# scientificcomputing/networks_fenicsx

Hardware: NVIDIA B200
Metric: tree-network assemble+solve DOFs/s (higher is better)
Workload: dtype f64

## Files before the change

networks_fenicsx_b200/csrc/assemble.cuh:

```cuda
#pragma once

#include "ctx.cuh"

namespace nxfx {

struct FastDiv {
  uint32_t magic, shift;
};
inline FastDiv make_fastdiv(uint32_t d) {
  FastDiv f;
  uint32_t fl = 31;
  while (!((d >> fl) & 1u)) --fl;
  if ((d & (d - 1)) == 0) {
    f.magic = 0;
    f.shift = fl == 0 ? 0 : fl - 1;
  } else {
    const uint64_t n = 1ull << (32 + fl);
    uint64_t m = n / d;
    const uint64_t rem = n % d;
    m += m;
    if (2 * rem >= d) m += 1;
    f.magic = (uint32_t)(m + 1);
    f.shift = fl;
  }
// ... 266 lines not shown
    for (int k = d.i0; k < d.i1; ++k) {
      const bool in = g.bif_inc[k] & 1;
      put(true, p, in ? 0.0 : -1.0);
      put(true, p + 1, in ? 1.0 : 0.0);
      p += 2;
    }
    if (rhs && !ACC) b[r] = 0.0;
  }
}

constexpr int kFluxRowsN1 = 512;
constexpr int kAsmCap = 2560;
constexpr int kPresRows = 512;
constexpr int kLamRows = 256;

#define NXFX_ST2(ptr, v) __stcs((ptr), (v))
#define NXFX_ST1(ptr, v) __stcs((ptr), (v))
#define NXFX_LDS(ptr) __ldcs(ptr)
#define NXFX_STB2(ptr, v) __stcs((ptr), (v))
#define NXFX_STB1(ptr, v) __stcs((ptr), (v))

template <bool ACC>
__device__ __forceinline__ void store_pair(double* __restrict__ vals, size_t idx, double v0, double v1) {
  if ((idx & 1) == 0) {
    double2* dst = reinterpret_cast<double2*>(vals + idx);
    double2 v = make_double2(v0, v1);
    if (ACC) { const double2 o = *dst; v.x += o.x; v.y += o.y; }
    NXFX_ST2(dst, v);
  } else {
    if (ACC) { vals[idx] += v0; vals[idx + 1] += v1; } else { vals[idx] = v0; vals[idx + 1] = v1; }
  }
}

template <bool ACC>
__device__ __forceinline__ void flush_tile(const double* sm, double* __restrict__ vals, int sbase, int tnnz) {
  const int off = sbase & 1;
  double* out = vals + sbase - off;
  const int lo = off, hi = off + tnnz;
  const int npair = (hi + 1) >> 1;
  for (int q = threadIdx.x; q < npair; q += blockDim.x) {
    const int i = 2 * q;
    if (i >= lo && i + 1 < hi) {
      double2 v = *reinterpret_cast<const double2*>(sm + i);
      double2* dst = reinterpret_cast<double2*>(out + i);
      if (ACC) { const double2 o = *dst; v.x += o.x; v.y += o.y; }
      NXFX_ST2(dst, v);
    } else {
      if (i >= lo && i < hi) { if (ACC) out[i] += sm[i]; else out[i] = sm[i]; }
      if (i + 1 >= lo && i + 1 < hi) { if (ACC) out[i + 1] += sm[i + 1]; else out[i + 1] = sm[i + 1]; }
    }
  }
}

template <bool ACC>
__device__ __forceinline__ void flux_tile_n1(const Net& g, const Coef& c, const int32_t* __restrict__ rowptr,
                                             double* __restrict__ vals, double* __restrict__ b, int lhs,
                                             int rhs, int tile, double* sm) {
  __shared__ int warp_nl[kTileRows / 32];
  const int r0 = tile * kFluxRowsN1;
  const int slot = (r0 >> 1) + threadIdx.x;
  const bool active = slot < g.E;
  const int lane = threadIdx.x & 31, w = threadIdx.x >> 5;
  int4 t = make_int4(0, 0, -1, -1);
  VertexRec v0, v1;
  if (active) {
    const int2 uv = NXFX_LDS(g.slot_uv + slot);
    v0 = load_vertex(g.x2, uv.x);
    v1 = load_vertex(g.x2, uv.y);
    t = make_int4(uv.x, uv.y, lm_unbox(v0.p), lm_unbox(v1.p));
  }
  const bool hu = t.z >= 0, hv = t.w >= 0;
  const unsigned bu = __ballot_sync(0xffffffffu, hu), bv = __ballot_sync(0xffffffffu, hv);
  const unsigned lt = (1u << lane) - 1u;
  int pre = __popc(bu & lt) + __popc(bv & lt);
  if (lane == 0) warp_nl[w] = __popc(bu) + __popc(bv);
  const int sbase = rowptr[r0];
  double m = 0.0;
  if (active) {
    const double R = c.R_cell ? c.R_cell[NXFX_LDS(g.slot_edge + slot)] : c.R_const;
    m = __dmul_rn(R, seg_length(v0, v1));
  }
  __syncthreads();
  int tot = 0;
#pragma unroll
  for (int k = 0; k < kTileRows / 32; ++k) {
    const int v = warp_nl[k];
    if (k < w) pre += v;
    tot += v;
  }
  const int nact = min(kFluxRowsN1 >> 1, g.E - (r0 >> 1));
  const int tnnz = 6 * nact + 2 * tot;
  if (active) {
    const int r = 2 * slot;
    if (rhs) {
      const double b0 = hu ? 0.0 : -v0.p, b1 = hv ? 0.0 : v1.p;
      double2* dst = reinterpret_cast<double2*>(b + r);
      double2 v = make_double2(b0, b1);
      if (ACC) { const double2 o = *dst; v.x += o.x; v.y += o.y; }
      NXFX_STB2(dst, v);
    }
    if (lhs) {
      if (ACC) c.cell_rh[slot] += m; else NXFX_STB1(c.cell_rh + slot, m);
      const double m3 = __dmul_rn(m, kThird), m6 = __dmul_rn(m, kSixth);
      const bool ufirst = !hv || (hu && t.z < t.w);
      const int nl = (int)hu + (int)hv;
      const double u0 = (hu && ufirst) ? -1.0 : 0.0, u1 = ufirst ? 0.0 : -1.0;
      const double w0 = (hu && ufirst) ? 0.0 : 1.0, w1 = ufirst ? 1.0 : 0.0;
      double* s0 = sm + (sbase & 1) + 6 * (int)threadIdx.x + 2 * pre;
      double* s1 = s0 + 3 + nl;
      s0[0] = m3; s0[1] = m6; s0[2] = 1.0;
      s1[0] = m6; s1[1] = m3; s1[2] = -1.0;
      if (nl > 0) { s0[3] = u0; s1[3] = w0; }
      if (nl > 1) { s0[4] = u1; s1[4] = w1; }
    }
  }
  if (lhs) {
    __syncthreads();
    flush_tile<ACC>(sm, vals, sbase, tnnz);
  }
}

template <bool ACC>
__device__ __forceinline__ void flux_tile_gen(const Net& g, const Coef& c, const int32_t* __restrict__ rowptr,
                                              double* __restrict__ vals, double* __restrict__ b, int lhs,
                                              int rhs, int tile, double* sm) {
  const int r0 = tile * kTileRows;
  const int rend = min(r0 + kTileRows, g.nq);
  const int r = r0 + threadIdx.x;
  RowDesc d;
  d.sbase = rowptr[r0];
  d.tnnz = rowptr[rend] - d.sbase;
  d.start = 0; d.a = 0; d.e = 0; d.i0 = d.i1 = 0;
  d.t = make_int4(0, 0, -1, -1);
  const bool active = r < rend;
  if (active) {
    d.start = rowptr[r] - d.sbase;
    const int slot = fastdiv(r, g.div_np1);
    d.a = r - slot * (g.N + 1);
    d.t = g.slot_uvl[slot];
    d.e = g.slot_edge[slot];
  }
  const int lane = threadIdx.x & 31;
  const int rr = active ? r : g.ndofs;
  if (d.tnnz > kAsmCap) {
    if (lhs) assemble_row<ACC, false>(g, c, d, rr, d.sbase + d.start, lane, b, lhs, rhs, GlobalSink<ACC>{vals});
    else assemble_row<ACC, false>(g, c, d, rr, 0, lane, b, lhs, rhs, [](bool, int, double) {});
    return;
  }
  assemble_row<ACC, false>(g, c, d, rr, (d.sbase & 1) + d.start, lane, b, lhs, rhs, SmemSink{sm});
  if (lhs) {
    __syncthreads();
    flush_tile<ACC>(sm, vals, d.sbase, d.tnnz);
  }
}

template <bool ACC, bool N1>
__device__ __forceinline__ void pressure_tile(const Net& g, const Coef& c, const int32_t* __restrict__ rowptr,
                                              double* __restrict__ vals, double* __restrict__ b, int lhs,
                                              int rhs, int tile) {
  const int r0 = g.poff + tile * kPresRows;
  const int rend = min(r0 + kPresRows, g.loff);
// ... 68 lines not shown
```

networks_fenicsx_b200/csrc/nxfx_b200.cu:

```cuda

#include <cub/device/device_scan.cuh>

#include <algorithm>
#include <atomic>
#include <chrono>
#include <cmath>
#include <cstdlib>

#include "assemble.cuh"
#include "ctx.cuh"
#include "condense.cuh"
#include "generic.cuh"
#include "precond.cuh"
#include "spmv.cuh"

using namespace nxfx;

namespace {

constexpr int kScalPartials = 8 * kMaxPartials;
constexpr int kScalSlots = 1024;

Net make_net(const nxfx_ctx* c) {
  Net g;
// ... 453 lines not shown
int cond_backward_local(nxfx_ctx* ctx, double* z, bool add) {
  Net g = make_net(ctx);
  CondDev c = make_cond(ctx);
  TreeDev t = make_tree(ctx);
  const int nb = ctx->tree.n_chunks - 1;
  if (ctx->n_bif > 0 && nb > 0) NXFX_LAUNCH(ctx, btree_sweep_kernel<2>, nb, 1024, 0, t, c, 0);
  const int grid = (int)cdiv((int64_t)ctx->E + ctx->n_bif, kCondThreads);
  if (add) NXFX_LAUNCH(ctx, cond_backsub_kernel<true>, grid, kCondThreads, 0, g, t, c, z);
  else NXFX_LAUNCH(ctx, cond_backsub_kernel<false>, grid, kCondThreads, 0, g, t, c, z);
  return NXFX_OK;
}

int do_cond_apply(nxfx_ctx* ctx, const double* r, double* z, bool add) {
  NXFX_REQUIRE(ctx, ctx->pc_ready, "pc_setup has not been run");
  int rc = cond_forward_local(ctx, r, nullptr);
  if (rc) return rc;
  if (ctx->n_bif > 0) NXFX_LAUNCH(ctx, btree_sweep_kernel<3>, 1, 1024, 0, make_tree(ctx), make_cond(ctx), ctx->tree.n_chunks - 1);
  return cond_backward_local(ctx, z, add);
}

bool n1_kernels(const nxfx_ctx* ctx) { return ctx->N == 1 && ctx->tree.fast_ok; }

int check_aligned(nxfx_ctx* ctx, const double* r, const double* z = nullptr) {
  NXFX_REQUIRE(ctx, (reinterpret_cast<uintptr_t>(r) & 15) == 0 && (reinterpret_cast<uintptr_t>(z) & 15) == 0,
               "vectors must be 16-byte aligned");
  return NXFX_OK;
}

int node_diag(nxfx_ctx* ctx, bool bif) {
  if (n1_kernels(ctx)) {
    if (bif) NXFX_LAUNCH(ctx, bif_diag_n1_kernel, (int)cdiv(ctx->n_bif, kThreads), kThreads, 0, make_net(ctx), make_tree(ctx), ctx->cur->cell_rh.p);
    return NXFX_OK;
  }
  NXFX_LAUNCH(ctx, edge_conductance_kernel, (int)cdiv(ctx->E, kThreads), kThreads, 0, ctx->E, ctx->N, ctx->cur->cell_rh.p, ctx->edge_g.p);
  if (bif) NXFX_LAUNCH(ctx, bif_diag_kernel, (int)cdiv(ctx->n_bif, kThreads), kThreads, 0, make_net(ctx), make_tree(ctx), ctx->edge_g.p);
  return NXFX_OK;
}

int node_rhs(nxfx_ctx* ctx, const double* r, bool bif) {
  Net g = make_net(ctx);
  TreeDev t = make_tree(ctx);
  if (n1_kernels(ctx)) {
    if (bif) NXFX_LAUNCH(ctx, bif_rhs_n1_kernel, (int)cdiv(ctx->n_bif, kThreads), kThreads, 0, g, t, r, ctx->cur->cell_rh.p, ctx->lam_weight.p);
    return NXFX_OK;
  }
  NXFX_LAUNCH(ctx, edge_condense_kernel<false>, (int)cdiv(ctx->E, kThreads), kThreads, 0, g, ctx->cur->cell_rh.p, r,
              ctx->edge_c.p, ctx->edge_fn.p, nullptr);
  if (bif)
    NXFX_LAUNCH(ctx, bif_rhs_kernel<false>, (int)cdiv(ctx->n_bif, kThreads), kThreads, 0, g, t, r, ctx->edge_g.p, ctx->edge_c.p,
                ctx->edge_fn.p, ctx->lam_weight.p);
  return NXFX_OK;
}

int edge_backsub(nxfx_ctx* ctx, const double* r, double* z, bool add, bool pdl = false) {
  Net g = make_net(ctx);
  TreeDev t = make_tree(ctx);
  const double* cell_rh = ctx->cur->cell_rh.p;
  const int grid = (int)cdiv((int64_t)ctx->E + ctx->n_bif, kThreads);
  if (!n1_kernels(ctx)) {
    if (add) NXFX_LAUNCH(ctx, edge_backsub_kernel<true>, grid, kThreads, 0, g, t, cell_rh, r, ctx->edge_g.p, ctx->edge_c.p, z);
    else NXFX_LAUNCH(ctx, edge_backsub_kernel<false>, grid, kThreads, 0, g, t, cell_rh, r, ctx->edge_g.p, ctx->edge_c.p, z);
    return NXFX_OK;
  }
  if (!pdl) {
    if (add) NXFX_LAUNCH(ctx, edge_backsub_n1_kernel<true>, grid, kThreads, 0, g, t, cell_rh, r, z);
    else NXFX_LAUNCH(ctx, edge_backsub_n1_kernel<false>, grid, kThreads, 0, g, t, cell_rh, r, z);
    return NXFX_OK;
  }
  cudaLaunchConfig_t cfg = {};
  cfg.gridDim = dim3((unsigned)grid);
  cfg.blockDim = dim3(kThreads);
  cfg.stream = ctx->stream;
  cudaLaunchAttribute attr[1];
  attr[0].id = cudaLaunchAttributeProgrammaticStreamSerialization;
  attr[0].val.programmaticStreamSerializationAllowed = 1;
  cfg.attrs = attr;
  cfg.numAttrs = 1;
  if (add) NXFX_CUDA(ctx, cudaLaunchKernelEx(&cfg, edge_backsub_n1_kernel<true>, g, t, cell_rh, r, z));
  else NXFX_CUDA(ctx, cudaLaunchKernelEx(&cfg, edge_backsub_n1_kernel<false>, g, t, cell_rh, r, z));
  ctx->launches++;
  return NXFX_OK;
}

int do_pc_setup(nxfx_ctx* ctx) {
  NXFX_REQUIRE(ctx, is_assembled(ctx), "assemble the matrix before pc_setup");
  if (ctx->generic) return do_cond_setup(ctx);
  NXFX_REQUIRE(ctx, ctx->tree.set, "nxfx_set_tree_schedule has not been called");
  const bool n1 = n1_kernels(ctx);
  int rc;
  if (!n1 && (rc = node_diag(ctx, ctx->n_bif > 0))) return rc;
  if (ctx->n_bif > 0 && (rc = tree_pass(ctx, true, nullptr, n1))) return rc;
  mark_factored(ctx);
  return NXFX_OK;
}

bool can_fuse_setup(const nxfx_ctx* ctx) {
  return !ctx->generic && ctx->tree.set && ctx->tree.fast_ok && ctx->tree.coop_fs_ok && ctx->n_bif > 0 &&
         ctx->tree.n_chunks > 1 && (!ctx->lam_weight.p || ctx->comm.ready) && ctx->cur->acc_count == 1;
}

int do_pc_setup_apply(nxfx_ctx* ctx, const double* r, double* z, bool add = false) {
  NXFX_REQUIRE(ctx, is_assembled(ctx), "assemble the matrix before pc_setup");
  const bool n1 = n1_kernels(ctx);
  if (n1) {
    int rc = check_aligned(ctx, r, z);
    if (rc) return rc;
  }
  auto& s = ctx->tree;
  Net g = make_net(ctx);
  TreeDev t = make_tree(ctx);
  FusedN1 fin{g, r, ctx->cur->cell_rh.p, ctx->lam_weight.p};
  unsigned int* tk = ctx->ticket.p + 1;
  unsigned int* fl = ctx->ticket.p + 2;
  unsigned int ep = ++s.epoch;
  int nb = s.n_chunks - 1;
  PeerDev pc = make_peer(ctx, 0);
  if (!n1) {
    NXFX_LAUNCH(ctx, edge_condense_kernel<true>, (int)cdiv(ctx->E, kThreads), kThreads, 0, g, ctx->cur->cell_rh.p, r,
                ctx->edge_c.p, ctx->edge_fn.p, ctx->edge_g.p);
    NXFX_LAUNCH(ctx, bif_rhs_kernel<true>, (int)cdiv(ctx->n_bif, kThreads), kThreads, 0, g, t, r, ctx->edge_g.p,
                ctx->edge_c.p, ctx->edge_fn.p, ctx->lam_weight.p);
    fin.r = nullptr;
    fin.cell_rh = nullptr;
  }
  cudaLaunchConfig_t cfg = {};
  const int gb = std::min(nb, s.coop_fs_blocks - 1);
  cfg.gridDim = dim3(gb + 1);
  cfg.blockDim = dim3(kTreeThreads);
  cfg.dynamicSmemBytes = tree_smem_bytes_fs(s.cap);
  cfg.stream = ctx->stream;
  cudaLaunchAttribute attr[2];
  attr[0].id = cudaLaunchAttributeCooperative;
  attr[0].val.cooperative = 1;
  attr[1].id = cudaLaunchAttributeProgrammaticStreamSerialization;
  attr[1].val.programmaticStreamSerializationAllowed = 1;
  cfg.attrs = attr;
  cfg.numAttrs = ctx->pdl_coop_refused ? 1 : 2;
  const bool multi = gb < nb;
  auto kern = pc.nranks > 1 ? (multi ? tree_factor_solve_coop_kernel<true, true> : tree_factor_solve_coop_kernel<true, false>)
                            : (multi ? tree_factor_solve_coop_kernel<false, true> : tree_factor_solve_coop_kernel<false, false>);
  cudaError_t le = cudaLaunchKernelEx(&cfg, kern, t, nb, tk, fl, ep, fin, pc);
  if (le != cudaSuccess && cfg.numAttrs == 2) {
    cudaGetLastError();
    ctx->pdl_coop_refused = true;
    cfg.numAttrs = 1;
    le = cudaLaunchKernelEx(&cfg, kern, t, nb, tk, fl, ep, fin, pc);
  }
  NXFX_CUDA(ctx, le);
  ctx->launches++;
  mark_factored(ctx);
  return edge_backsub(ctx, r, z, add, true);
}

int do_pc_apply(nxfx_ctx* ctx, int pc_type, const double* r, double* z, bool add = false) {
  const int n = (int)ctx->ndofs;
  if (pc_type == NXFX_PC_NETWORK_SCHUR && ctx->cur->acc_count > 1 && !ctx->pc_unscaled) {
    const size_t ld = vec_stride(ctx);
    if (ctx->work2.n < 2 * ld) {
      NXFX_CUDA(ctx, cudaStreamSynchronize(ctx->stream));
      NXFX_CUDA(ctx, ctx->work2.alloc(2 * ld));
    }
    const double inv_k = 1.0 / (double)ctx->cur->acc_count;
    double* rs = ctx->work2.p;
    double* zs = ctx->work2.p + ld;
    NXFX_LAUNCH(ctx, scale_tail_kernel<false>, vec_grid(ctx, n), kThreads, 0, n, (int)ctx->poff, inv_k, r, rs);
    ctx->pc_unscaled = true;
    const int rc = do_pc_apply(ctx, pc_type, rs, zs, false);
    ctx->pc_unscaled = false;
    if (rc) return rc;
    if (add) NXFX_LAUNCH(ctx, scale_tail_kernel<true>, vec_grid(ctx, n), kThreads, 0, n, (int)ctx->poff, inv_k, zs, z);
    else NXFX_LAUNCH(ctx, scale_tail_kernel<false>, vec_grid(ctx, n), kThreads, 0, n, (int)ctx->poff, inv_k, zs, z);
    return NXFX_OK;
  }
  if (add && pc_type != NXFX_PC_NETWORK_SCHUR) {
    int rc = ensure_work(ctx, 3);
    if (rc) return rc;
    double* tmp = ctx->work.p + 2 * vec_stride(ctx);
    if ((rc = do_pc_apply(ctx, pc_type, r, tmp, false))) return rc;
    NXFX_LAUNCH(ctx, add_kernel, vec_grid(ctx, n), kThreads, 0, n, tmp, z);
    return NXFX_OK;
  }
  if (ctx->comm.ready) {
    NXFX_REQUIRE(ctx, pc_type == NXFX_PC_NETWORK_SCHUR && can_fuse_setup(ctx),
                 "the fused partitioned solve needs a forest schedule that fits the cooperative kernel and pc_type lu");
    return do_pc_setup_apply(ctx, r, z, add);
  }
  if (pc_type == NXFX_PC_NONE) {
    NXFX_CUDA(ctx, cudaMemcpyAsync(z, r, n * sizeof(double), cudaMemcpyDeviceToDevice, ctx->stream));
    return NXFX_OK;
  }
  if (pc_type == NXFX_PC_JACOBI_FLUX) {
    NXFX_LAUNCH(ctx, jacobi_flux_kernel, (int)cdiv(n, kThreads), kThreads, 0, n, (int)ctx->nq,
                ctx->rowptr.p, ctx->colidx.p, ctx->cur->vals.p, r, z);
    return NXFX_OK;
  }
  NXFX_REQUIRE(ctx, ctx->pc_ready, "pc_setup has not been run");
  if (ctx->generic) return do_cond_apply(ctx, r, z, add);
  const bool n1 = n1_kernels(ctx);
  int rc;
  if (n1 && (rc = check_aligned(ctx, r, z))) return rc;
  const bool fuse = n1 && ctx->n_bif > 0 && ctx->tree.coop_ok && ctx->tree.n_chunks > 1 && !ctx->lam_weight.p;
  if ((rc = node_rhs(ctx, r, ctx->n_bif > 0 && !fuse))) return rc;
  if (ctx->n_bif > 0 && (rc = tree_pass(ctx, false, r, fuse))) return rc;
  return edge_backsub(ctx, r, z, add);
}

int factor_bottom(nxfx_ctx* ctx) {
  if (ctx->generic) return cond_factor_local(ctx);
  int rc = node_diag(ctx, true);
  if (rc) return rc;
  const int nb = ctx->tree.n_chunks - 1;
  if (nb > 0) NXFX_LAUNCH(ctx, tree_factor_kernel, nb, kTreeThreads, tree_smem_bytes(ctx->tree.cap), make_tree(ctx), nb, ctx->ticket.p + 1, 0,
                          (FusedN1{make_net(ctx), nullptr, nullptr}));
  return NXFX_OK;
}

int forward_bottom(nxfx_ctx* ctx, const double* r) {
  if (ctx->generic) return cond_forward_local(ctx, r, ctx->lam_weight.p);
  int rc = node_rhs(ctx, r, true);
  if (rc) return rc;
  const int nb = ctx->tree.n_chunks - 1;
  if (nb > 0) NXFX_LAUNCH(ctx, tree_solve_kernel<kTreeUp>, nb, kTreeThreads, tree_smem_bytes(ctx->tree.cap), make_tree(ctx), nb, ctx->ticket.p + 1, 0);
  return NXFX_OK;
}

template <bool FACTOR, int PHASE>
int top_split(nxfx_ctx* ctx, double* buf) {
  const int top = ctx->tree.n_chunks - 1;
  if (!ctx->generic) {
    NXFX_LAUNCH(ctx, (tree_top_kernel<FACTOR, PHASE>), 1, kTreeThreads, tree_smem_bytes(ctx->tree.cap), make_tree(ctx), top, buf);
    return NXFX_OK;
  }
  if (ctx->n_bif == 0) return NXFX_OK;
  const int32_t* idx = ctx->n_shared > 0 ? ctx->top_sh_idx.p : nullptr;
  NXFX_LAUNCH(ctx, (btree_top_split_kernel<FACTOR, PHASE>), 1, 1024, 0, make_tree(ctx), make_cond(ctx), top, idx,
              std::max(ctx->n_shared, 1), buf);
  return NXFX_OK;
}

int backward_bottom(nxfx_ctx* ctx, const double* r, double* z, bool add) {
  if (ctx->generic) return cond_backward_local(ctx, z, add);
  const int nb = ctx->tree.n_chunks - 1;
  if (nb > 0) NXFX_LAUNCH(ctx, tree_solve_kernel<kTreeDown>, nb, kTreeThreads, tree_smem_bytes(ctx->tree.cap), make_tree(ctx), nb, ctx->ticket.p + 1, 0);
  return edge_backsub(ctx, r, z, add);
}

bool fused_split(const nxfx_ctx* ctx) { return !ctx->generic && n1_kernels(ctx); }

int pack_shared(nxfx_ctx* ctx, const double* r, const double* b, double* buf, bool cont) {
  const int ns = ctx->n_shared;
  if (ns == 0) return NXFX_OK;
  NXFX_LAUNCH(ctx, pack_shared_kernel, (int)cdiv(ns, kThreads), kThreads, 0, ns, (int)ctx->loff, ctx->shared_lm.p, r, buf);
  if (!cont) return NXFX_OK;
  NXFX_LAUNCH(ctx, pack_nodal_kernel, (int)cdiv(ns, kThreads), kThreads, 0, ns, (int)ctx->nq, ctx->shared_lm.p, ctx->cond.bif_node.p,
              r, buf + ns);
  NXFX_LAUNCH(ctx, pack_nodal_kernel, (int)cdiv(ns, kThreads), kThreads, 0, ns, (int)ctx->nq, ctx->shared_lm.p, ctx->cond.bif_node.p,
              b, buf + 2 * (size_t)ns);
  return NXFX_OK;
}

inline size_t vec_stride(const nxfx_ctx* ctx) { return ((size_t)ctx->ndofs + 1) & ~(size_t)1; }

int ensure_work(nxfx_ctx* ctx, size_t nvec) {
  const size_t need = nvec * vec_stride(ctx);
  if (ctx->work.n >= need) return NXFX_OK;
  NXFX_CUDA(ctx, cudaStreamSynchronize(ctx->stream));
  NXFX_CUDA(ctx, ctx->work.alloc(need));
  return NXFX_OK;
}

inline double kNormSentinel() {
  const uint64_t bits = 0x7FF8DEADBEEF0001ull;
  double d;
  std::memcpy(&d, &bits, sizeof d);
  return d;
}
inline bool is_norm_sentinel(double v) {
  uint64_t bits;
  std::memcpy(&bits, &v, sizeof bits);
  return bits == 0x7FF8DEADBEEF0001ull;
}
bool poll_norms_enabled() {
  static const bool on = [] { const char* e = std::getenv("NXFX_POLL_NORMS"); return !(e && e[0] == '0'); }();
  return on;
}

void push_history(nxfx_solve_info* info, double v) {
  if (info->history_len < NXFX_HISTORY_LEN) info->history[info->history_len++] = v;
}

int mirror_copy(nxfx_ctx* ctx, const double* x) {
  if (!ctx->mirror_h) return NXFX_OK;
  NXFX_CUDA(ctx, cudaEventRecord(ctx->ev_x, ctx->stream));
  NXFX_CUDA(ctx, cudaStreamWaitEvent(ctx->side, ctx->ev_x, 0));
  NXFX_CUDA(ctx, cudaMemcpyAsync(ctx->mirror_h, x, (size_t)ctx->ndofs * sizeof(double), cudaMemcpyDeviceToHost, ctx->side));
  return NXFX_OK;
}

int solve_preonly(nxfx_ctx* ctx, const double* b, double* x, const nxfx_solve_opts* o, nxfx_solve_info* info,
                  bool fused_setup) {
  int rc = ensure_work(ctx, 3);
  if (rc) return rc;
  double* r = ctx->work.p;
  const int steps = std::max(0, std::min(o->refine_steps, 32));
  if ((rc = fused_setup ? do_pc_setup_apply(ctx, b, x) : do_pc_apply(ctx, o->pc_type, b, x, false))) return rc;
  if ((rc = mirror_copy(ctx, x))) return rc;
  info->iterations = 1;
  if (steps == 0 && !o->final_residual) {
    NXFX_CUDA(ctx, cudaStreamSynchronize(ctx->stream));
    info->rhs_norm = info->residual_norm = -1.0;
    info->converged = 1;
    return NXFX_OK;
  }
  const double rt = o->refine_rtol > 0.0 ? o->refine_rtol : 0.0;
  int applied = 0;
  while (true) {
    const bool lazy = ctx->pipe_ok;
    volatile double* nh = ctx->scal_h;
    const bool poll = poll_norms_enabled();
    if (poll) { ctx->scal_h[0] = kNormSentinel(); ctx->scal_h[1] = kNormSentinel(); }
    if ((rc = do_residual(ctx, b, x, lazy ? nullptr : r, ctx->scal_h_dev, true))) return rc;
    bool arrived = false;
    if (poll) {
      const auto t0 = std::chrono::steady_clock::now();
      for (unsigned spin = 0;; ++spin) {
        if (!is_norm_sentinel(nh[0]) && !is_norm_sentinel(nh[1])) { arrived = true; break; }
        if ((spin & 255u) == 255u && std::chrono::steady_clock::now() - t0 > std::chrono::microseconds(1500)) break;
      }
      std::atomic_thread_fence(std::memory_order_acquire);
    }
    if (!arrived) NXFX_CUDA(ctx, cudaStreamSynchronize(ctx->stream));
    info->rhs_norm = std::sqrt(ctx->scal_h[1]);
    info->residual_norm = std::sqrt(ctx->scal_h[0]);
    push_history(info, info->residual_norm);
    const bool good = std::isfinite(info->residual_norm) && info->residual_norm <= rt * info->rhs_norm;
    if (applied >= steps || (good && rt > 0.0) || !std::isfinite(info->residual_norm)) break;
    if (lazy && (rc = do_residual(ctx, b, x, r, slot(ctx, 0)))) return rc;
    if ((rc = do_pc_apply(ctx, o->pc_type, r, x, true))) return rc;
    if ((rc = mirror_copy(ctx, x))) return rc;
    ++applied;
    if (applied >= steps && !o->final_residual) break;
  }
  info->iterations = 1 + applied;
  const double tol = std::max(o->rtol * info->rhs_norm, o->atol);
  info->converged = std::isfinite(info->residual_norm) && info->residual_norm <= tol;
  return NXFX_OK;
}

int solve_fgmres(nxfx_ctx* ctx, const double* b, double* x, const nxfx_solve_opts* o, nxfx_solve_info* info) {
  const int n = (int)ctx->ndofs;
  const int m = std::max(1, std::min(o->restart > 0 ? o->restart : 30, 200));
  NXFX_REQUIRE(ctx, 2 * (m + 2) + 8 < kScalSlots, "restart too large");
  int rc = ensure_work(ctx, (size_t)(2 * m + 3));
  if (rc) return rc;
  const size_t ld = vec_stride(ctx);
  double* V = ctx->work.p;
  double* Z = V + (size_t)(m + 1) * ld;
  double* w = Z + (size_t)m * ld;
  double* r = w + ld;
  double* hcol = slot(ctx, 8);
  double* hcol2 = slot(ctx, 8 + m + 2);
  double* ycoef = slot(ctx, 8 + 2 * (m + 2));
  std::vector<double> H((size_t)(m + 1) * m, 0.0), cs(m), sn(m), gvec(m + 1), y(m);

  NXFX_CUDA(ctx, cudaMemsetAsync(x, 0, n * sizeof(double), ctx->stream));
  int its = 0;
  const int max_it = o->max_it > 0 ? o->max_it : 10000;
  double tol = 0.0;
  while (true) {
    if ((rc = do_residual(ctx, b, x, r, slot(ctx, 1)))) return rc;
    NXFX_CUDA(ctx, cudaMemcpyAsync(ctx->scal_h, slot(ctx, 1), 2 * sizeof(double), cudaMemcpyDeviceToHost, ctx->stream));
    NXFX_CUDA(ctx, cudaStreamSynchronize(ctx->stream));
    info->rhs_norm = std::sqrt(ctx->scal_h[1]);
    const double beta = std::sqrt(ctx->scal_h[0]);
// ... 1082 lines not shown
```

networks_fenicsx_b200/csrc/precond.cuh:

```cuda
#pragma once

#include "assemble.cuh"
#include "peer.cuh"
#include "spmv.cuh"

namespace nxfx {

struct TreeDev {
  const int32_t* __restrict__ t_of_bif;
  const int32_t* __restrict__ bif_of_t;
  const int32_t* __restrict__ t_parent;
  const int32_t* __restrict__ t_pedge;
  const int32_t* __restrict__ t_pslot;
  const int32_t* __restrict__ t_cptr;
  const int32_t* __restrict__ t_cidx;
  const int32_t* __restrict__ chunk_lptr;
  const int32_t* __restrict__ lvl_ptr;
  const int32_t* __restrict__ chunk_desc;
  const int32_t* __restrict__ t_inc_ptr;
  const int2* __restrict__ t_inc;
  double* diag0;
  double* tg;
  double* d;
  double* gd;
// ... 1048 lines not shown
  const double* rq = r + (size_t)slot * (N + 1);
  const double* rp = r + g.poff + (size_t)e * N;
  const double* rh = cell_rh + (size_t)e * N;
  double* zq = z + (size_t)slot * (N + 1);
  double* zp = z + g.poff + (size_t)e * N;
  const double q0 = edge_g[e] * (edge_c[e] + lu - lv);
  double F = 0.0, qprev = 0.0, qa = q0, hl = 0.0, p = lu;
  for (int a = 0; a <= N; ++a) {
    if (ADD) zq[a] += qa; else zq[a] = qa;
    double qn = 0.0, hr = 0.0;
    if (a < N) {
      F += rp[a];
      qn = q0 + F;
      hr = rh[a];
      const double Mq = hl * (qprev * kSixth + qa * kThird) + hr * (qa * kThird + qn * kSixth);
      p += rq[a] - Mq;
      if (ADD) zp[a] += p; else zp[a] = p;
    }
    qprev = qa;
    qa = qn;
    hl = hr;
  }
}

__global__ void __launch_bounds__(kThreads)
bif_diag_n1_kernel(Net g, TreeDev t, const double* __restrict__ cell_rh) {
  const int i = blockIdx.x * blockDim.x + threadIdx.x;
  if (i >= g.n_bif) return;
  double s = 0.0;
  for (int k = g.bif_ptr[i]; k < g.bif_ptr[i + 1]; ++k) s += 1.0 / cell_rh[g.edge_slot[g.bif_inc[k] >> 1]];
  const int n = t.t_of_bif[i];
  t.diag0[n] = s;
  const int pe = t.t_pslot[n];
  t.tg[n] = pe >= 0 ? 1.0 / cell_rh[pe] : 0.0;
}

__global__ void __launch_bounds__(kThreads)
bif_rhs_n1_kernel(Net g, TreeDev t, const double* __restrict__ r, const double* __restrict__ cell_rh,
                  const double* __restrict__ lam_weight) {
  const int i = blockIdx.x * blockDim.x + threadIdx.x;
  if (i >= g.n_bif) return;
  double s = lam_weight ? -lam_weight[i] * r[g.loff + i] : -r[g.loff + i];
  for (int k = g.bif_ptr[i]; k < g.bif_ptr[i + 1]; ++k) {
    const int inc = g.bif_inc[k], e = inc >> 1;
    const int slot = g.edge_slot[e];
    const double2 rq = *reinterpret_cast<const double2*>(r + 2 * (size_t)slot);
    const double rp = r[g.poff + e], rh = cell_rh[slot];
    const double gc = (1.0 / rh) * (rq.x + rq.y) - 0.5 * rp;
    s += (inc & 1) ? (rp + gc) : -gc;
  }
  t.r[t.t_of_bif[i]] = s;
}

template <bool ADD>
__global__ void __launch_bounds__(kThreads)
edge_backsub_n1_kernel(Net g, TreeDev t, const double* __restrict__ cell_rh, const double* __restrict__ r,
                       double* __restrict__ z) {
  asm volatile("griddepcontrol.launch_dependents;");
  const int idx = blockIdx.x * blockDim.x + threadIdx.x;
  if (idx >= g.E) {
    asm volatile("griddepcontrol.wait;" ::: "memory");
    const int i = idx - g.E;
    if (i < g.n_bif) { if (ADD) z[g.loff + i] += t.lam_nat[i]; else z[g.loff + i] = t.lam_nat[i]; }
    return;
  }
  const int slot = idx;
  const int4 uv = g.slot_uvl[slot];
  const int e = g.slot_edge[slot];
  const double2 rq = *reinterpret_cast<const double2*>(r + 2 * (size_t)slot);
  const double rp = r[g.poff + e], rh = cell_rh[slot];
  asm volatile("griddepcontrol.wait;" ::: "memory");
  const double lu = uv.z >= 0 ? t.lam_nat[uv.z] : 0.0;
  const double lv = uv.w >= 0 ? t.lam_nat[uv.w] : 0.0;
  const double c = (rq.x + rq.y) - 0.5 * rh * rp;
  const double q0 = (c + lu - lv) / rh;
  const double q1 = q0 + rp;
  const double p = lu + rq.x - rh * (q0 * kThird + q1 * kSixth);
  double2* zq = reinterpret_cast<double2*>(z + 2 * (size_t)slot);
  if (ADD) {
    const double2 o = *zq;
    *zq = make_double2(o.x + q0, o.y + q1);
    z[g.poff + e] += p;
  } else {
    *zq = make_double2(q0, q1);
    z[g.poff + e] = p;
  }
}

__global__ void __launch_bounds__(kThreads)
pack_shared_kernel(int n_shared, int loff, const int32_t* __restrict__ shared_lm,
                   const double* __restrict__ v, double* __restrict__ buf) {
  const int i = blockIdx.x * blockDim.x + threadIdx.x;
  if (i < n_shared) buf[i] = v[loff + shared_lm[i]];
}

__global__ void __launch_bounds__(kThreads)
residual_finish_kernel(int n_shared, int loff, const int32_t* __restrict__ shared_lm,
                       const double* __restrict__ buf, double* __restrict__ r, double* __restrict__ nrm_out) {
  __shared__ double red[kThreads / 32];
  double acc = 0.0;
  for (int i = threadIdx.x; i < n_shared; i += blockDim.x) {
    const double v = buf[i];
    r[loff + shared_lm[i]] = v;
    acc += v * v;
  }
  acc = warp_sum(acc);
  if ((threadIdx.x & 31) == 0) red[threadIdx.x >> 5] = acc;
  __syncthreads();
  if (threadIdx.x == 0) {
    double s = buf[n_shared];
    for (int w = 0; w < kThreads / 32; ++w) s += red[w];
    nrm_out[0] = s;
    nrm_out[1] = buf[n_shared + 1];
  }
}

__global__ void __launch_bounds__(kThreads)
jacobi_flux_kernel(int n, int nq, const int32_t* __restrict__ rowptr,
                   const int32_t* __restrict__ colidx, const double* __restrict__ vals,
                   const double* __restrict__ r, double* __restrict__ z) {
  const int i = blockIdx.x * blockDim.x + threadIdx.x;
  if (i >= n) return;
  double v = r[i];
  if (i < nq) {
    for (int k = rowptr[i]; k < rowptr[i + 1]; ++k)
      if (colidx[k] == i) v /= vals[k];
  }
  z[i] = v;
}

}
```

networks_fenicsx_b200/csrc/spmv.cuh:

```cuda
#pragma once

#include "ctx.cuh"
#include "peer.cuh"

namespace nxfx {

constexpr int kEntriesPerThread = kTileCap / kTileRows;
constexpr int kMaxPartials = 4096;

__device__ __forceinline__ double warp_sum(double v) {
#pragma unroll
  for (int o = 16; o > 0; o >>= 1) v += __shfl_down_sync(0xffffffffu, v, o);
  return v;
}

template <int THREADS>
__device__ __forceinline__ double block_sum(double v, double* red ) {
  v = warp_sum(v);
  const int lane = threadIdx.x & 31, w = threadIdx.x >> 5;
  if (lane == 0) red[w] = v;
  __syncthreads();
  double s = 0.0;
  if (w == 0) {
    s = lane < THREADS / 32 ? red[lane] : 0.0;
    s = warp_sum(s);
  }
  __syncthreads();
  return s;
}

template <int THREADS, int K>
__device__ __forceinline__ bool finish_partials(double (&mine)[K], double* partial, int nblocks,
                                                unsigned int* ticket, double* out, double* red) {
  __shared__ bool last;
  if (threadIdx.x == 0) {
#pragma unroll
    for (int k = 0; k < K; ++k) partial[(size_t)k * kMaxPartials + blockIdx.x] = mine[k];
    __threadfence();
    const unsigned int t = atomicAdd(ticket, 1u);
    last = (t == (unsigned int)nblocks - 1);
  }
  __syncthreads();
  if (!last) return false;
  __threadfence();
#pragma unroll
  for (int k = 0; k < K; ++k) {
    double s = 0.0;
    for (int i = threadIdx.x; i < nblocks; i += THREADS)
      s += ((volatile double*)partial)[(size_t)k * kMaxPartials + i];
    s = block_sum<THREADS>(s, red);
    if (threadIdx.x == 0) out[k] = s;
  }
  if (threadIdx.x == 0) *ticket = 0u;
  return true;
}

template <int MODE>
__global__ void __launch_bounds__(kTileRows)
spmv_kernel(int n, int ntiles, const int32_t* __restrict__ rowptr,
            const int32_t* __restrict__ colidx, const double* __restrict__ vals,
            const double* __restrict__ x, double* __restrict__ y, const double* __restrict__ b,
            double* partial, unsigned int* ticket, double* norm2_out) {
  __shared__ double sm[kTileCap];
  __shared__ int srow[kTileRows + 1];
  __shared__ double red[kTileRows / 32];
  double nrm = 0.0, nrb = 0.0;
  for (int tile = blockIdx.x; tile < ntiles; tile += gridDim.x) {
    const int r0 = tile * kTileRows;
    const int nr = min(kTileRows, n - r0);
    if (threadIdx.x <= nr) srow[threadIdx.x] = rowptr[r0 + threadIdx.x];
    if (threadIdx.x == 0) srow[nr] = rowptr[r0 + nr];
    __syncthreads();
    const int sbase = srow[0];
    const int tnnz = srow[nr] - sbase;
    const bool valid = threadIdx.x < nr;
    const int rs = valid ? srow[threadIdx.x] - sbase : 0;
    const int re = valid ? srow[threadIdx.x + 1] - sbase : 0;
    double acc = 0.0;
    for (int c0 = 0; c0 < tnnz; c0 += kTileCap) {
      const int cnt = min(kTileCap, tnnz - c0);
      const size_t g0 = (size_t)sbase + c0;
      double v[kEntriesPerThread];
      int c[kEntriesPerThread];
#pragma unroll
      for (int k = 0; k < kEntriesPerThread; ++k) {
        const int idx = threadIdx.x + k * kTileRows;
        if (idx < cnt) {
          v[k] = __ldg(vals + g0 + idx);
          c[k] = __ldg(colidx + g0 + idx);
        }
      }
#pragma unroll
      for (int k = 0; k < kEntriesPerThread; ++k) {
        const int idx = threadIdx.x + k * kTileRows;
        if (idx < cnt) sm[idx] = __dmul_rn(v[k], x[c[k]]);
      }
      __syncthreads();
      const int s = max(rs - c0, 0), e = min(re - c0, cnt);
      for (int k = s; k < e; ++k) acc = __dadd_rn(acc, sm[k]);
      __syncthreads();
    }
    if (valid) {
      if (MODE == 0) {
        y[r0 + threadIdx.x] = acc;
      } else {
        const double bi = b[r0 + threadIdx.x];
        const double r = __dsub_rn(bi, acc);
        y[r0 + threadIdx.x] = r;
        nrm += r * r;
        nrb += bi * bi;
      }
    }
  }
  if (MODE == 1) {
    double mine[2] = {block_sum<kTileRows>(nrm, red), block_sum<kTileRows>(nrb, red)};
    finish_partials<kTileRows, 2>(mine, partial, gridDim.x, ticket, norm2_out, red);
  }
}

constexpr int kPipeCap = 1792;
#ifndef NXFX_SPMV_STAGES
#define NXFX_SPMV_STAGES 2
#endif
constexpr int kStages = NXFX_SPMV_STAGES;

struct alignas(128) SpmvStage {
  double vals[kPipeCap];
  int cols[kPipeCap];
  int rows[kTileRows + 8];
};

__device__ __forceinline__ uint32_t smem_u32(const void* p) {
  return (uint32_t)__cvta_generic_to_shared(p);
}
__device__ __forceinline__ void mbar_init(uint64_t* bar, uint32_t count) {
  asm volatile("mbarrier.init.shared::cta.b64 [%0], %1;" ::"r"(smem_u32(bar)), "r"(count));
}
__device__ __forceinline__ void mbar_expect_tx(uint64_t* bar, uint32_t bytes) {
  asm volatile("mbarrier.arrive.expect_tx.shared::cta.b64 _, [%0], %1;" ::"r"(smem_u32(bar)), "r"(bytes)
               : "memory");
}
__device__ __forceinline__ uint64_t l2_evict_first_policy() {
  uint64_t p;
  asm volatile("createpolicy.fractional.L2::evict_first.b64 %0, 1.0;" : "=l"(p));
  return p;
}
__device__ __forceinline__ void bulk_g2s_stream(void* dst, const void* src, uint32_t bytes, uint64_t* bar,
                                                uint64_t policy) {
  asm volatile(
      "cp.async.bulk.shared::cluster.global.mbarrier::complete_tx::bytes.L2::cache_hint [%0], [%1], %2, [%3], %4;" ::"r"(
          smem_u32(dst)),
      "l"(src), "r"(bytes), "r"(smem_u32(bar)), "l"(policy)
      : "memory");
}
__device__ __forceinline__ void mbar_wait(uint64_t* bar, uint32_t parity) {
  uint32_t ok = 0;
  const uint32_t addr = smem_u32(bar);
  while (!ok) {
    asm volatile(
        "{\n.reg .pred p;\nmbarrier.try_wait.parity.shared::cta.b64 p, [%1], %2;\nselp.u32 %0, 1, 0, p;\n}"
        : "=r"(ok)
        : "r"(addr), "r"(parity)
        : "memory");
  }
}

__global__ void __launch_bounds__(kThreads)
tile_base_kernel(int n, int ntiles, const int32_t* __restrict__ rowptr, int32_t* __restrict__ tile_base,
                 int32_t* __restrict__ max_tile_nnz) {
  const int t = blockIdx.x * blockDim.x + threadIdx.x;
// ... 220 lines not shown
```

Before: 21.38 billion.

## Fuse first refinement residual into edge back-substitution and lambda-row kernel

When refinement or a final residual is requested, the edge back-substitution kernel also computes the edge rows of the residual norm. It reads the freshly assembled matrix tile via bulk async copy and multiplies it with the just-solved q/p/lambda values in registers. A separate PDL-chained kernel handles the lambda (bifurcation) rows and finishes the partial-sum reduction, so the first full SpMV residual pass is skipped. This adds extra matrix reads and reduction work to the back-substitution and relies on the n1 layout assumptions matching the assembly.

```diff
diff --git a/networks_fenicsx_b200/csrc/assemble.cuh b/networks_fenicsx_b200/csrc/assemble.cuh
--- a/networks_fenicsx_b200/csrc/assemble.cuh
+++ b/networks_fenicsx_b200/csrc/assemble.cuh
@@ -342,15 +342,43 @@
   }
 }
 
+struct FluxRowsN1 {
+  int off;
+  int nl;
+  bool ufirst;
+  int tnnz;
+};
+__device__ __forceinline__ FluxRowsN1 flux_rows_n1(int lm_u, int lm_v, int nact) {
+  __shared__ int warp_nl[kTileRows / 32];
+  const int lane = threadIdx.x & 31, w = threadIdx.x >> 5;
+  const bool hu = lm_u >= 0, hv = lm_v >= 0;
+  const unsigned bu = __ballot_sync(0xffffffffu, hu), bv = __ballot_sync(0xffffffffu, hv);
+  const unsigned lt = (1u << lane) - 1u;
+  int pre = __popc(bu & lt) + __popc(bv & lt);
+  if (lane == 0) warp_nl[w] = __popc(bu) + __popc(bv);
+  __syncthreads();
+  int tot = 0;
+#pragma unroll
+  for (int k = 0; k < kTileRows / 32; ++k) {
+    const int v = warp_nl[k];
+    if (k < w) pre += v;
+    tot += v;
+  }
+  FluxRowsN1 L;
+  L.off = 6 * (int)threadIdx.x + 2 * pre;
+  L.nl = (int)hu + (int)hv;
+  L.ufirst = !hv || (hu && lm_u < lm_v);
+  L.tnnz = 6 * nact + 2 * tot;
+  return L;
+}
+
 template <bool ACC>
 __device__ __forceinline__ void flux_tile_n1(const Net& g, const Coef& c, const int32_t* __restrict__ rowptr,
                                              double* __restrict__ vals, double* __restrict__ b, int lhs,
                                              int rhs, int tile, double* sm) {
-  __shared__ int warp_nl[kTileRows / 32];
   const int r0 = tile * kFluxRowsN1;
   const int slot = (r0 >> 1) + threadIdx.x;
   const bool active = slot < g.E;
-  const int lane = threadIdx.x & 31, w = threadIdx.x >> 5;
   int4 t = make_int4(0, 0, -1, -1);
   VertexRec v0, v1;
   if (active) {
@@ -360,26 +388,14 @@
     t = make_int4(uv.x, uv.y, lm_unbox(v0.p), lm_unbox(v1.p));
   }
   const bool hu = t.z >= 0, hv = t.w >= 0;
-  const unsigned bu = __ballot_sync(0xffffffffu, hu), bv = __ballot_sync(0xffffffffu, hv);
-  const unsigned lt = (1u << lane) - 1u;
-  int pre = __popc(bu & lt) + __popc(bv & lt);
-  if (lane == 0) warp_nl[w] = __popc(bu) + __popc(bv);
   const int sbase = rowptr[r0];
   double m = 0.0;
   if (active) {
     const double R = c.R_cell ? c.R_cell[NXFX_LDS(g.slot_edge + slot)] : c.R_const;
     m = __dmul_rn(R, seg_length(v0, v1));
   }
-  __syncthreads();
-  int tot = 0;
-#pragma unroll
-  for (int k = 0; k < kTileRows / 32; ++k) {
-    const int v = warp_nl[k];
-    if (k < w) pre += v;
-    tot += v;
-  }
-  const int nact = min(kFluxRowsN1 >> 1, g.E - (r0 >> 1));
-  const int tnnz = 6 * nact + 2 * tot;
+  const FluxRowsN1 L = flux_rows_n1(t.z, t.w, min(kFluxRowsN1 >> 1, g.E - (r0 >> 1)));
+  const int tnnz = L.tnnz;
   if (active) {
     const int r = 2 * slot;
     if (rhs) {
@@ -392,11 +408,11 @@
     if (lhs) {
       if (ACC) c.cell_rh[slot] += m; else NXFX_STB1(c.cell_rh + slot, m);
       const double m3 = __dmul_rn(m, kThird), m6 = __dmul_rn(m, kSixth);
-      const bool ufirst = !hv || (hu && t.z < t.w);
-      const int nl = (int)hu + (int)hv;
+      const bool ufirst = L.ufirst;
+      const int nl = L.nl;
       const double u0 = (hu && ufirst) ? -1.0 : 0.0, u1 = ufirst ? 0.0 : -1.0;
       const double w0 = (hu && ufirst) ? 0.0 : 1.0, w1 = ufirst ? 1.0 : 0.0;
-      double* s0 = sm + (sbase & 1) + 6 * (int)threadIdx.x + 2 * pre;
+      double* s0 = sm + (sbase & 1) + L.off;
       double* s1 = s0 + 3 + nl;
       s0[0] = m3; s0[1] = m6; s0[2] = 1.0;
       s1[0] = m6; s1[1] = m3; s1[2] = -1.0;
diff --git a/networks_fenicsx_b200/csrc/nxfx_b200.cu b/networks_fenicsx_b200/csrc/nxfx_b200.cu
--- a/networks_fenicsx_b200/csrc/nxfx_b200.cu
+++ b/networks_fenicsx_b200/csrc/nxfx_b200.cu
@@ -529,18 +529,24 @@
   return NXFX_OK;
 }
 
-int edge_backsub(nxfx_ctx* ctx, const double* r, double* z, bool add, bool pdl = false) {
+int check_edge_grid(const nxfx_ctx* ctx) { return (int)std::min<int64_t>(cdiv(ctx->E, kThreads), kMaxPartials / 2); }
+int check_lambda_grid(const nxfx_ctx* ctx) { return (int)std::min<int64_t>(cdiv(ctx->n_bif, kTileRows), kMaxPartials / 2); }
+
+int edge_backsub(nxfx_ctx* ctx, const double* r, double* z, bool add, bool pdl = false, double* check_norm2 = nullptr) {
   Net g = make_net(ctx);
   TreeDev t = make_tree(ctx);
   const double* cell_rh = ctx->cur->cell_rh.p;
-  const int grid = (int)cdiv((int64_t)ctx->E + ctx->n_bif, kThreads);
+  const int grid = check_norm2 ? check_edge_grid(ctx) : (int)cdiv((int64_t)ctx->E + ctx->n_bif, kThreads);
   if (!n1_kernels(ctx)) {
     if (add) NXFX_LAUNCH(ctx, edge_backsub_kernel<true>, grid, kThreads, 0, g, t, cell_rh, r, ctx->edge_g.p, ctx->edge_c.p, z);
     else NXFX_LAUNCH(ctx, edge_backsub_kernel<false>, grid, kThreads, 0, g, t, cell_rh, r, ctx->edge_g.p, ctx->edge_c.p, z);
     return NXFX_OK;
   }
   if (!pdl) {
-    if (add) NXFX_LAUNCH(ctx, edge_backsub_n1_kernel<true>, grid, kThreads, 0, g, t, cell_rh, r, z);
+    if (check_norm2)
+      NXFX_LAUNCH(ctx, edge_backsub_residual_n1_kernel, grid, kThreads, 0, g, t, cell_rh, r, ctx->rowptr.p, ctx->cur->vals.p, z,
+                  ctx->scal.p, ctx->ticket.p, check_norm2);
+    else if (add) NXFX_LAUNCH(ctx, edge_backsub_n1_kernel<true>, grid, kThreads, 0, g, t, cell_rh, r, z);
     else NXFX_LAUNCH(ctx, edge_backsub_n1_kernel<false>, grid, kThreads, 0, g, t, cell_rh, r, z);
     return NXFX_OK;
   }
@@ -553,8 +559,29 @@
   attr[0].val.programmaticStreamSerializationAllowed = 1;
   cfg.attrs = attr;
   cfg.numAttrs = 1;
-  if (add) NXFX_CUDA(ctx, cudaLaunchKernelEx(&cfg, edge_backsub_n1_kernel<true>, g, t, cell_rh, r, z));
+  if (check_norm2)
+    NXFX_CUDA(ctx, cudaLaunchKernelEx(&cfg, edge_backsub_residual_n1_kernel, g, t, cell_rh, r, (const int32_t*)ctx->rowptr.p,
+                                      (const double*)ctx->cur->vals.p, z, ctx->scal.p, ctx->ticket.p, check_norm2));
+  else if (add) NXFX_CUDA(ctx, cudaLaunchKernelEx(&cfg, edge_backsub_n1_kernel<true>, g, t, cell_rh, r, z));
   else NXFX_CUDA(ctx, cudaLaunchKernelEx(&cfg, edge_backsub_n1_kernel<false>, g, t, cell_rh, r, z));
+  ctx->launches++;
+  return NXFX_OK;
+}
+
+int lambda_residual(nxfx_ctx* ctx, const double* b, const double* x, double* norm2_d) {
+  if (ctx->n_bif == 0) return NXFX_OK;
+  cudaLaunchConfig_t cfg = {};
+  cfg.gridDim = dim3((unsigned)check_lambda_grid(ctx));
+  cfg.blockDim = dim3(kTileRows);
+  cfg.stream = ctx->stream;
+  cudaLaunchAttribute attr[1];
+  attr[0].id = cudaLaunchAttributeProgrammaticStreamSerialization;
+  attr[0].val.programmaticStreamSerializationAllowed = 1;
+  cfg.attrs = attr;
+  cfg.numAttrs = 1;
+  NXFX_CUDA(ctx, cudaLaunchKernelEx(&cfg, lambda_residual_kernel, (int)ctx->ndofs, (int)ctx->loff, (const int32_t*)ctx->rowptr.p,
+                                    (const int32_t*)ctx->colidx.p, (const double*)ctx->cur->vals.p, x, b, ctx->scal.p,
+                                    check_edge_grid(ctx), ctx->ticket.p, norm2_d));
   ctx->launches++;
   return NXFX_OK;
 }
@@ -576,7 +603,7 @@
          ctx->tree.n_chunks > 1 && (!ctx->lam_weight.p || ctx->comm.ready) && ctx->cur->acc_count == 1;
 }
 
-int do_pc_setup_apply(nxfx_ctx* ctx, const double* r, double* z, bool add = false) {
+int do_pc_setup_apply(nxfx_ctx* ctx, const double* r, double* z, bool add = false, double* check_norm2 = nullptr) {
   NXFX_REQUIRE(ctx, is_assembled(ctx), "assemble the matrix before pc_setup");
   const bool n1 = n1_kernels(ctx);
   if (n1) {
@@ -626,10 +653,10 @@
   NXFX_CUDA(ctx, le);
   ctx->launches++;
   mark_factored(ctx);
-  return edge_backsub(ctx, r, z, add, true);
-}
-
-int do_pc_apply(nxfx_ctx* ctx, int pc_type, const double* r, double* z, bool add = false) {
+  return edge_backsub(ctx, r, z, add, true, check_norm2);
+}
+
+int do_pc_apply(nxfx_ctx* ctx, int pc_type, const double* r, double* z, bool add = false, double* check_norm2 = nullptr) {
   const int n = (int)ctx->ndofs;
   if (pc_type == NXFX_PC_NETWORK_SCHUR && ctx->cur->acc_count > 1 && !ctx->pc_unscaled) {
     const size_t ld = vec_stride(ctx);
@@ -679,7 +706,7 @@
   const bool fuse = n1 && ctx->n_bif > 0 && ctx->tree.coop_ok && ctx->tree.n_chunks > 1 && !ctx->lam_weight.p;
   if ((rc = node_rhs(ctx, r, ctx->n_bif > 0 && !fuse))) return rc;
   if (ctx->n_bif > 0 && (rc = tree_pass(ctx, false, r, fuse))) return rc;
-  return edge_backsub(ctx, r, z, add);
+  return edge_backsub(ctx, r, z, add, false, check_norm2);
 }
 
 int factor_bottom(nxfx_ctx* ctx) {
@@ -774,14 +801,26 @@
   return NXFX_OK;
 }
 
+bool fused_check(const nxfx_ctx* ctx, const nxfx_solve_opts* o) {
+  return o->pc_type == NXFX_PC_NETWORK_SCHUR && !ctx->generic && n1_kernels(ctx) && !ctx->comm.ready &&
+         !ctx->lam_weight.p && ctx->cur->acc_count == 1;
+}
+
 int solve_preonly(nxfx_ctx* ctx, const double* b, double* x, const nxfx_solve_opts* o, nxfx_solve_info* info,
                   bool fused_setup) {
   int rc = ensure_work(ctx, 3);
   if (rc) return rc;
   double* r = ctx->work.p;
   const int steps = std::max(0, std::min(o->refine_steps, 32));
-  if ((rc = fused_setup ? do_pc_setup_apply(ctx, b, x) : do_pc_apply(ctx, o->pc_type, b, x, false))) return rc;
+  const bool fused = (steps > 0 || o->final_residual) && fused_check(ctx, o);
+  volatile double* nh = ctx->scal_h;
+  const bool poll = poll_norms_enabled();
+  auto arm = [&] { if (poll) { ctx->scal_h[0] = kNormSentinel(); ctx->scal_h[1] = kNormSentinel(); } };
+  if (fused) arm();
+  double* chk = fused ? ctx->scal_h_dev : nullptr;
+  if ((rc = fused_setup ? do_pc_setup_apply(ctx, b, x, false, chk) : do_pc_apply(ctx, o->pc_type, b, x, false, chk))) return rc;
   if ((rc = mirror_copy(ctx, x))) return rc;
+  if (fused && (rc = lambda_residual(ctx, b, x, ctx->scal_h_dev))) return rc;
   info->iterations = 1;
   if (steps == 0 && !o->final_residual) {
     NXFX_CUDA(ctx, cudaStreamSynchronize(ctx->stream));
@@ -792,11 +831,12 @@
   const double rt = o->refine_rtol > 0.0 ? o->refine_rtol : 0.0;
   int applied = 0;
   while (true) {
-    const bool lazy = ctx->pipe_ok;
-    volatile double* nh = ctx->scal_h;
-    const bool poll = poll_norms_enabled();
-    if (poll) { ctx->scal_h[0] = kNormSentinel(); ctx->scal_h[1] = kNormSentinel(); }
-    if ((rc = do_residual(ctx, b, x, lazy ? nullptr : r, ctx->scal_h_dev, true))) return rc;
+    const bool fused_now = fused && applied == 0;
+    const bool lazy = ctx->pipe_ok || fused_now;
+    if (!fused_now) {
+      arm();
+      if ((rc = do_residual(ctx, b, x, lazy ? nullptr : r, ctx->scal_h_dev, true))) return rc;
+    }
     bool arrived = false;
     if (poll) {
       const auto t0 = std::chrono::steady_clock::now();
diff --git a/networks_fenicsx_b200/csrc/precond.cuh b/networks_fenicsx_b200/csrc/precond.cuh
--- a/networks_fenicsx_b200/csrc/precond.cuh
+++ b/networks_fenicsx_b200/csrc/precond.cuh
@@ -1124,6 +1124,15 @@
   t.r[t.t_of_bif[i]] = s;
 }
 
+struct EdgeN1 { double q0, q1, p; };
+__device__ __forceinline__ EdgeN1 edge_solve_n1(double2 rq, double rp, double rh, double lu, double lv) {
+  const double c = (rq.x + rq.y) - 0.5 * rh * rp;
+  const double q0 = (c + lu - lv) / rh;
+  const double q1 = q0 + rp;
+  const double p = lu + rq.x - rh * (q0 * kThird + q1 * kSixth);
+  return {q0, q1, p};
+}
+
 template <bool ADD>
 __global__ void __launch_bounds__(kThreads)
 edge_backsub_n1_kernel(Net g, TreeDev t, const double* __restrict__ cell_rh, const double* __restrict__ r,
@@ -1144,18 +1153,105 @@
   asm volatile("griddepcontrol.wait;" ::: "memory");
   const double lu = uv.z >= 0 ? t.lam_nat[uv.z] : 0.0;
   const double lv = uv.w >= 0 ? t.lam_nat[uv.w] : 0.0;
-  const double c = (rq.x + rq.y) - 0.5 * rh * rp;
-  const double q0 = (c + lu - lv) / rh;
-  const double q1 = q0 + rp;
-  const double p = lu + rq.x - rh * (q0 * kThird + q1 * kSixth);
+  const EdgeN1 s = edge_solve_n1(rq, rp, rh, lu, lv);
   double2* zq = reinterpret_cast<double2*>(z + 2 * (size_t)slot);
   if (ADD) {
     const double2 o = *zq;
-    *zq = make_double2(o.x + q0, o.y + q1);
-    z[g.poff + e] += p;
+    *zq = make_double2(o.x + s.q0, o.y + s.q1);
+    z[g.poff + e] += s.p;
   } else {
-    *zq = make_double2(q0, q1);
-    z[g.poff + e] = p;
+    *zq = make_double2(s.q0, s.q1);
+    z[g.poff + e] = s.p;
+  }
+}
+
+__global__ void __launch_bounds__(kThreads)
+edge_backsub_residual_n1_kernel(Net g, TreeDev t, const double* __restrict__ cell_rh, const double* __restrict__ b,
+                                const int32_t* __restrict__ rowptr, const double* __restrict__ vals,
+                                double* __restrict__ x, double* partial, unsigned int* ticket, double* norm2_out) {
+  __shared__ __align__(16) double sv[kAsmCap + 2];
+  __shared__ double red[kThreads / 32];
+  __shared__ uint64_t full;
+  asm volatile("griddepcontrol.launch_dependents;");
+  const int tid = threadIdx.x;
+  if (tid == 0) {
+    mbar_init(&full, 1);
+    asm volatile("fence.mbarrier_init.release.cluster;" ::: "memory");
+    asm volatile("fence.proxy.async.shared::cta;" ::: "memory");
+  }
+  const uint64_t stream_policy = l2_evict_first_policy();
+  const int ntiles = (g.E + kThreads - 1) / kThreads;
+  const double* pvals = vals + rowptr[g.poff];
+  double nrm = 0.0, nrb = 0.0;
+  uint32_t parity = 0;
+  for (int tile = blockIdx.x; tile < ntiles; tile += gridDim.x, parity ^= 1u) {
+    const int slot = tile * kThreads + tid;
+    const bool active = slot < g.E;
+    const int r0 = tile * kFluxRowsN1;
+    const int sbase = rowptr[r0];
+    const int off = sbase & 1;
+    if (tid == 0) {
+      const int send = rowptr[min(r0 + kFluxRowsN1, g.nq)];
+      const uint32_t bytes = (uint32_t)((off + send - sbase + 1) >> 1) * 16u;
+      mbar_expect_tx(&full, bytes);
+      bulk_g2s_stream(sv, vals + sbase - off, bytes, &full, stream_policy);
+    }
+    int4 uv = make_int4(0, 0, -1, -1);
+    int e = 0;
+    double2 bq = make_double2(0.0, 0.0), pv = make_double2(0.0, 0.0);
+    double bp = 0.0, rh = 0.0;
+    if (active) {
+      uv = g.slot_uvl[slot];
+      e = g.slot_edge[slot];
+      bq = *reinterpret_cast<const double2*>(b + 2 * (size_t)slot);
+      bp = b[g.poff + e];
+      rh = cell_rh[slot];
+      pv = make_double2(__ldcs(pvals + 2 * (size_t)e), __ldcs(pvals + 2 * (size_t)e + 1));
+    }
+    const FluxRowsN1 L = flux_rows_n1(uv.z, uv.w, min(kThreads, g.E - tile * kThreads));
+    mbar_wait(&full, parity);
+    asm volatile("griddepcontrol.wait;" ::: "memory");
+    if (active) {
+      const double lu = uv.z >= 0 ? t.lam_nat[uv.z] : 0.0;
+      const double lv = uv.w >= 0 ? t.lam_nat[uv.w] : 0.0;
+      const EdgeN1 s = edge_solve_n1(bq, bp, rh, lu, lv);
+      *reinterpret_cast<double2*>(x + 2 * (size_t)slot) = make_double2(s.q0, s.q1);
+      x[g.poff + e] = s.p;
+      const double* a0 = sv + off + L.off;
+      const double* a1 = a0 + 3 + L.nl;
+      const double la = L.ufirst ? lu : lv, lb = L.ufirst ? lv : lu;
+      double au = 0.0, av = 0.0, ap = 0.0;
+      au = __dadd_rn(au, __dmul_rn(a0[0], s.q0));
+      av = __dadd_rn(av, __dmul_rn(a1[0], s.q0));
+      ap = __dadd_rn(ap, __dmul_rn(pv.x, s.q0));
+      au = __dadd_rn(au, __dmul_rn(a0[1], s.q1));
+      av = __dadd_rn(av, __dmul_rn(a1[1], s.q1));
+      ap = __dadd_rn(ap, __dmul_rn(pv.y, s.q1));
+      au = __dadd_rn(au, __dmul_rn(a0[2], s.p));
+      av = __dadd_rn(av, __dmul_rn(a1[2], s.p));
+      if (L.nl > 0) {
+        au = __dadd_rn(au, __dmul_rn(a0[3], la));
+        av = __dadd_rn(av, __dmul_rn(a1[3], la));
+      }
+      if (L.nl > 1) {
+        au = __dadd_rn(au, __dmul_rn(a0[4], lb));
+        av = __dadd_rn(av, __dmul_rn(a1[4], lb));
+      }
+      const double ru = __dsub_rn(bq.x, au), rv = __dsub_rn(bq.y, av), rp = __dsub_rn(bp, ap);
+      nrm += ru * ru + rv * rv + rp * rp;
+      nrb += bq.x * bq.x + bq.y * bq.y + bp * bp;
+    }
+    asm volatile("fence.proxy.async.shared::cta;" ::: "memory");
+    __syncthreads();
+  }
+  asm volatile("griddepcontrol.wait;" ::: "memory");
+  for (int i = blockIdx.x * kThreads + tid; i < g.n_bif; i += gridDim.x * kThreads) x[g.loff + i] = t.lam_nat[i];
+  double mine[2] = {block_sum<kThreads>(nrm, red), block_sum<kThreads>(nrb, red)};
+  if (g.n_bif == 0) {
+    finish_partials<kThreads, 2>(mine, partial, gridDim.x, ticket, norm2_out, red);
+  } else if (tid == 0) {
+    partial[blockIdx.x] = mine[0];
+    partial[kMaxPartials + blockIdx.x] = mine[1];
   }
 }
 
diff --git a/networks_fenicsx_b200/csrc/spmv.cuh b/networks_fenicsx_b200/csrc/spmv.cuh
--- a/networks_fenicsx_b200/csrc/spmv.cuh
+++ b/networks_fenicsx_b200/csrc/spmv.cuh
@@ -31,11 +31,11 @@
 
 template <int THREADS, int K>
 __device__ __forceinline__ bool finish_partials(double (&mine)[K], double* partial, int nblocks,
-                                                unsigned int* ticket, double* out, double* red) {
+                                                unsigned int* ticket, double* out, double* red, int first = 0) {
   __shared__ bool last;
   if (threadIdx.x == 0) {
 #pragma unroll
-    for (int k = 0; k < K; ++k) partial[(size_t)k * kMaxPartials + blockIdx.x] = mine[k];
+    for (int k = 0; k < K; ++k) partial[(size_t)k * kMaxPartials + first + blockIdx.x] = mine[k];
     __threadfence();
     const unsigned int t = atomicAdd(ticket, 1u);
     last = (t == (unsigned int)nblocks - 1);
@@ -46,7 +46,7 @@
 #pragma unroll
   for (int k = 0; k < K; ++k) {
     double s = 0.0;
-    for (int i = threadIdx.x; i < nblocks; i += THREADS)
+    for (int i = threadIdx.x; i < first + nblocks; i += THREADS)
       s += ((volatile double*)partial)[(size_t)k * kMaxPartials + i];
     s = block_sum<THREADS>(s, red);
     if (threadIdx.x == 0) out[k] = s;
@@ -116,6 +116,64 @@
     double mine[2] = {block_sum<kTileRows>(nrm, red), block_sum<kTileRows>(nrb, red)};
     finish_partials<kTileRows, 2>(mine, partial, gridDim.x, ticket, norm2_out, red);
   }
+}
+
+__global__ void __launch_bounds__(kTileRows)
+lambda_residual_kernel(int n, int loff, const int32_t* __restrict__ rowptr, const int32_t* __restrict__ colidx,
+                       const double* __restrict__ vals, const double* __restrict__ x, const double* __restrict__ b,
+                       double* partial, int first, unsigned int* ticket, double* norm2_out) {
+  __shared__ double sm[kTileCap];
+  __shared__ int srow[kTileRows + 1];
+  __shared__ double red[kTileRows / 32];
+  const int tid = threadIdx.x;
+  const int ntiles = (n - loff + kTileRows - 1) / kTileRows;
+  double nrm = 0.0, nrb = 0.0;
+  for (int tile = blockIdx.x; tile < ntiles; tile += gridDim.x) {
+    const int r0 = loff + tile * kTileRows;
+    const int nr = min(kTileRows, n - r0);
+    if (tid < nr) srow[tid] = rowptr[r0 + tid];
+    if (tid == 0) srow[nr] = rowptr[r0 + nr];
+    const double bi = tid < nr ? __ldcs(b + r0 + tid) : 0.0;
+    __syncthreads();
+    const int sbase = srow[0];
+    const int tnnz = srow[nr] - sbase;
+    const int rs = tid < nr ? srow[tid] - sbase : 0;
+    const int re = tid < nr ? srow[tid + 1] - sbase : 0;
+    double acc = 0.0;
+    for (int c0 = 0; c0 < tnnz; c0 += kTileCap) {
+      const int cnt = min(kTileCap, tnnz - c0);
+      const size_t g0 = (size_t)sbase + c0;
+      double v[kEntriesPerThread];
+      int c[kEntriesPerThread];
+#pragma unroll
+      for (int k = 0; k < kEntriesPerThread; ++k) {
+        const int idx = tid + k * kTileRows;
+        if (idx < cnt) {
+          v[k] = __ldcs(vals + g0 + idx);
+          c[k] = __ldcs(colidx + g0 + idx);
+        }
+      }
+      asm volatile("griddepcontrol.wait;" ::: "memory");
+#pragma unroll
+      for (int k = 0; k < kEntriesPerThread; ++k) {
+        const int idx = tid + k * kTileRows;
+        if (idx < cnt) sm[idx] = __dmul_rn(v[k], x[c[k]]);
+      }
+      __syncthreads();
+      const int s = max(rs - c0, 0), e = min(re - c0, cnt);
+      for (int k = s; k < e; ++k) acc = __dadd_rn(acc, sm[k]);
+      __syncthreads();
+    }
+    if (tid < nr) {
+      const double r = __dsub_rn(bi, acc);
+      nrm += r * r;
+      nrb += bi * bi;
+    }
+    __syncthreads();
+  }
+  asm volatile("griddepcontrol.wait;" ::: "memory");
+  double mine[2] = {block_sum<kTileRows>(nrm, red), block_sum<kTileRows>(nrb, red)};
+  finish_partials<kTileRows, 2>(mine, partial, gridDim.x, ticket, norm2_out, red, first);
 }
 
 constexpr int kPipeCap = 1792;
```

Result: faster. 21.74 billion (median of 6 runs) (+1.7%).
